# theori-io/nrsc5

Measured on AMD Instinct MI355X. Metric: IQ MS/s demod+decoded, higher is better.
Workload: dtype exact float32 half-band (== int16 Q15) / f32 OFDM + sync / int32 Viterbi metrics

## Files before the change

### nrsc5_amd/build.py

```python
from __future__ import annotations

import contextlib
import fcntl
import os
import subprocess
import sys

ROOT = os.path.dirname(os.path.dirname(os.path.abspath(__file__)))
CSRC = os.path.join(ROOT, "nrsc5_amd", "csrc")
HIP_SOURCES = ["engine.hip", "k_decimate.hip", "k_acquire.hip", "k_mixfft.hip", "k_sync.hip", "k_decode.hip", "k_replay.hip", "k_trim.hip", "k_am.hip", "k_l2.hip", "hdc_consumer.hip", "k_channelize.hip", "k_scan.hip"]
LIB = os.path.join(ROOT, "nrsc5_amd", "libnrsc5hip.so")
EMU_LIB = os.path.join(ROOT, "tests", "simt", "libnrsc5hip_emu.so")
HIPCC = os.environ.get("HIPCC", "/opt/rocm/bin/hipcc")


def _stale(target: str, deps) -> bool:
    if not os.path.exists(target):
        return True
    t = os.path.getmtime(target)
    return any(os.path.getmtime(d) > t for d in deps)


def _deps():
    d = [os.path.join(CSRC, f) for f in os.listdir(CSRC)]
    d.append(os.path.join(ROOT, "include", "nrsc5hip.h"))
    return d


@contextlib.contextmanager
def _build_lock(target: str):
    fd = os.open(os.path.dirname(target), os.O_RDONLY)
    try:
        fcntl.flock(fd, fcntl.LOCK_EX)
        yield
    finally:
        os.close(fd)


def _compile_to(target: str, cmd_for) -> None:
    tmp = "%s.tmp%d" % (target, os.getpid())
    try:
        subprocess.check_call(cmd_for(tmp))
        os.replace(tmp, target)
    finally:
        if os.path.exists(tmp):
            os.unlink(tmp)


def source_sha() -> str:
    import hashlib
    h = hashlib.sha256()
    for f in sorted(_deps()):
        if f.endswith((".hip", ".h")):
            h.update(os.path.basename(f).encode()); h.update(open(f, "rb").read())
    return h.hexdigest()[:16]


def build_hip(force: bool = False, verbose: bool = False) -> str:
    if force or _stale(LIB, _deps()):
        with _build_lock(LIB):
            if force or _stale(LIB, _deps()):
                srcs = [os.path.join(CSRC, f) for f in HIP_SOURCES if os.path.exists(os.path.join(CSRC, f))]

                def cmd(out):
                    c = [HIPCC, "--offload-arch=gfx950", "-O3", "-std=c++17", "-fPIC", "-shared", "-ffp-contract=off",
                         '-DNRSC5HIP_SOURCE_SHA="%s"' % source_sha(),
                         "-I" + os.path.join(ROOT, "include"), "-I" + CSRC, "-o", out] + srcs
                    if verbose:
                        print(" ".join(c))
                    return c
                _compile_to(LIB, cmd)
    return LIB


def build_hip_diag(flags, out_name: str) -> str:
    out = os.path.join(ROOT, "nrsc5_amd", out_name)
    srcs = [os.path.join(CSRC, f) for f in HIP_SOURCES if os.path.exists(os.path.join(CSRC, f))]
    cmd = [HIPCC, "--offload-arch=gfx950", "-O3", "-std=c++17", "-fPIC", "-shared", "-ffp-contract=off", '-DNRSC5HIP_SOURCE_SHA="%s"' % source_sha(),
           "-I" + os.path.join(ROOT, "include"), "-I" + CSRC, "-o", out] + list(flags) + srcs
    subprocess.check_call(cmd)
    return out


def _host_has_fma() -> bool:
    try:
        flags = next(l for l in open("/proc/cpuinfo") if l.startswith("flags")).split()
    except (OSError, StopIteration):
        return False
    return "fma" in flags


def build_emu(force: bool = False) -> str:
    simt = os.path.join(ROOT, "tests", "simt")
    deps = _deps() + [os.path.join(simt, "hipemu.h"), os.path.join(simt, "hipemu.cpp")]
    if force or _stale(EMU_LIB, deps):
        with _build_lock(EMU_LIB):
            if force or _stale(EMU_LIB, deps):
                srcs = [os.path.join(CSRC, f) for f in HIP_SOURCES if os.path.exists(os.path.join(CSRC, f))]
                fma = ["-mfma"] if _host_has_fma() else []

                def cmd(out):
                    c = ["g++", "-O2", "-g", "-std=c++17", "-fPIC", "-shared", "-ffp-contract=off", "-w"] + fma + ['-DNRSC5HIP_SOURCE_SHA="%s"' % source_sha(),
                         "-I" + simt, "-I" + os.path.join(ROOT, "include"), "-I" + CSRC, "-o", out,
                         os.path.join(simt, "hipemu.cpp")]
                    for s in srcs:
                        c += ["-x", "c++", s]
                    return c
                _compile_to(EMU_LIB, cmd)
    return EMU_LIB


if __name__ == "__main__":
    if "--emu" in sys.argv:
        print(build_emu(force=True))
    elif "--accurate-trig" in sys.argv:
        print(build_hip_diag(["-DNRSC5HIP_ACCURATE_TRIG"], "libnrsc5hip_acctrig.so"))
    elif "--cmul-unfused" in sys.argv:
        print(build_hip_diag(["-DNRSC5HIP_CMUL_UNFUSED"], "libnrsc5hip_unfused.so"))
    elif "--mixfft-noload" in sys.argv:
        print(build_hip_diag(["-DNRSC5HIP_MIXFFT_NOLOAD"], "libnrsc5hip_noload.so"))
    elif "--mixfft-phases" in sys.argv:
        print(build_hip_diag(["-DNRSC5HIP_MIXFFT_PHASES"], "libnrsc5hip_mixphases.so"))
    else:
        print(build_hip(force=True, verbose=True))
```

### nrsc5_amd/csrc/k_decode.hip

```cpp
#include <hip/hip_runtime.h>
#include "kernels.h"
#include "viterbi_wave.h"
#include "viterbi_v3.h"
#include "l2_header.h"

namespace nrsc5 {

__device__ inline int stream_of(const int *ids, int idx) { return ids ? ids[idx] : idx; }

__global__ __launch_bounds__(256) void k_p1_deint(DevTables tb, DevBuffers db, const int *ids, int parity, int lane_id)
{
    const int s = stream_of(ids, blockIdx.y);
    StreamState &st = db.state[s];
    if (!st.p1_pending[parity]) return;
    __shared__ uint32_t tile[16 * 180];
    __shared__ uint16_t lut[384];
    const int r = blockIdx.x, tid = threadIdx.x;
    const int8_t *pm = db.pm + ((size_t)s * NPM + st.p1_pmslot[parity]) * PM_FRAME;
    uint32_t *out = (uint32_t *)(db.coded + ((size_t)lane_id * db.nstreams_alloc + s) * P1_LEN);
    for (int w = tid; w < 16 * 180; w += 256) {
        const int b = w / 180, x = w % 180;
        tile[w] = ((const uint32_t *)(pm + ((size_t)b * 32 + r) * 720))[x];
    }
    for (int q = tid; q < 384; q += 256) lut[q] = tb.deint_lut[q];
    __syncthreads();
    const uint8_t *bytes = (const uint8_t *)tile;
    const int k0 = (3 * r) & 31;
    const int nk = (P1_CODED / 320 - k0 + 31) / 32;
    for (int idx = tid; idx < nk * 128; idx += 256) {
        const int m = idx >> 7, i = idx & 127;
        const int k = k0 + 32 * m;
        const int col = (11 * k + k / 288) % 36;
        uint32_t v = 0;
#pragma unroll
        for (int t = 0; t < 3; t++) {
            const unsigned off = lut[3 * i + t];
            if (off != 0xffffu) v |= (uint32_t)bytes[off + col] << (8 * t);
        }
        out[128 * k + i] = v;
    }
}

__device__ inline int bit_errors_k7_at(const int *soft, const uint32_t *bits, int len, int i)
{
    unsigned r = 0;
#pragma unroll
    for (int k = 0; k < 7; k++) {
        int q = i - k; if (q < 0) q += len;
        r |= ((bits[q >> 5] >> (q & 31)) & 1u) << (6 - k);
    }
    const int w = soft[i];
    const int c0 = (int8_t)w, c1 = (int8_t)(w >> 8), c2 = (int8_t)(w >> 16);
    const int p0 = __popc(r & 0133u) & 1, p1 = __popc(r & 0171u) & 1, p2 = __popc(r & 0165u) & 1;
    return ((c0 > 0) != p0) + ((c1 > 0) != p1) + (((i & 1) == 0) && ((c2 > 0) != p2));
}

__device__ inline int bit_errors_k7_partial(const int *soft, const uint32_t *bits, int len)
{
    int errors = 0;
    for (int i = threadIdx.x; i < len; i += blockDim.x) {
        unsigned r = 0;
#pragma unroll
        for (int k = 0; k < 7; k++) {
            int q = i - k; if (q < 0) q += len;
            r |= ((bits[q >> 5] >> (q & 31)) & 1u) << (6 - k);
        }
        const int w = soft[i];
        const int c0 = (int8_t)w, c1 = (int8_t)(w >> 8), c2 = (int8_t)(w >> 16);
        const int p0 = __popc(r & 0133u) & 1, p1 = __popc(r & 0171u) & 1, p2 = __popc(r & 0165u) & 1;
        if ((c0 > 0) != p0) errors++;
        if ((c1 > 0) != p1) errors++;
        if ((i & 1) == 0 && ((c2 > 0) != p2)) errors++;
    }
    return errors;
}

constexpr int FWD_WAVES = 4;
__global__ __launch_bounds__(64 * FWD_WAVES) void k_p1_forward(DevTables tb, DevBuffers db, const int *ids, int parity, int lane_id, int prio, int nstreams, int G, int warm)
{
    wave_set_priority(prio);
    const int widx = wave_uniform((int)(blockIdx.x * FWD_WAVES + (threadIdx.x >> 6)));
    if (widx >= nstreams * G) return;
    const int sidx = widx / G, g = widx % G;
    const int s = wave_uniform(stream_of(ids, sidx));
    StreamState &st = db.state[s];
    if (!st.p1_pending[parity]) return;
    const size_t slot = (size_t)lane_id * db.nstreams_alloc + s;
    const int *soft = db.coded + slot * P1_LEN;
    uint32_t *dec = db.dec + slot * (size_t)(2 * (P1_LEN + 64));
    viterbi3_forward_segment(soft, P1_LEN, dec, db.fwd_meta + slot * (size_t)(VIT3_GMAX * VIT3_META), g, G, warm);
}

__global__ __launch_bounds__(64 * FWD_WAVES) void k_p1_fix(DevTables tb, DevBuffers db, const int *ids, int parity, int lane_id, int prio, int nstreams, int G)
{
    wave_set_priority(prio);
    const int sidx = wave_uniform((int)(blockIdx.x * FWD_WAVES + (threadIdx.x >> 6)));
    if (sidx >= nstreams) return;
    const int s = wave_uniform(stream_of(ids, sidx));
    StreamState &st = db.state[s];
    if (!st.p1_pending[parity]) return;
    const size_t slot = (size_t)lane_id * db.nstreams_alloc + s;
    const int endlane = viterbi3_forward_fix(db.coded + slot * P1_LEN, P1_LEN, db.dec + slot * (size_t)(2 * (P1_LEN + 64)),
                                             db.fwd_meta + slot * (size_t)(VIT3_GMAX * VIT3_META), G, db.fwd_stats);
    if ((threadIdx.x & 63) == 0) st.p1_endlane[parity] = endlane;
}

constexpr int TB_THREADS = 1024;
constexpr int TBM_WAVES = 4;

__global__ __launch_bounds__(64 * TBM_WAVES) void k_p1_tbmap(DevTables tb, DevBuffers db, const int *ids, int parity, int lane_id, int prio, int parts)
{
    wave_set_priority(prio);
    const int s = stream_of(ids, blockIdx.y);
    StreamState &st = db.state[s];
    if (!st.p1_pending[parity]) return;
    const size_t slot = (size_t)lane_id * db.nstreams_alloc + s;
    viterbi3_traceback_maps(db.dec + slot * (size_t)(2 * (P1_LEN + 64)), P1_LEN, db.tbmap + slot * ((size_t)(P1_LEN / 64 + 1) * 64),
                            (int)(blockIdx.x * TBM_WAVES + (threadIdx.x >> 6)), parts * TBM_WAVES);
}

__global__ __launch_bounds__(64) void k_p1_tbwalk(DevTables tb, DevBuffers db, const int *ids, int parity, int lane_id, int prio, int nparts, int ntasks)
{
    wave_set_priority(prio);
    __shared__ uint32_t lds[TB2_LDS_WORDS];
    for (int t = (int)blockIdx.x; t < ntasks; t += (int)gridDim.x) {
        const int s = wave_uniform(stream_of(ids, t / nparts));
        StreamState &st = db.state[s];
        if (!st.p1_pending[parity]) continue;
        const size_t slot = (size_t)lane_id * db.nstreams_alloc + s;
        uint32_t *out = db.p1_ring + ((size_t)s * db.p1_slots + st.p1_slot[parity]) * P1_WORDS;
        viterbi3_traceback_walk(db.dec + slot * (size_t)(2 * (P1_LEN + 64)), P1_LEN, st.p1_endlane[parity], out,
                                db.tbmap + slot * ((size_t)(P1_LEN / 64 + 1) * 64), t % nparts, lds, db.coded + slot * P1_LEN);
        WAVE_LDS_FENCE();
    }
}

__global__ __launch_bounds__(TB_THREADS) void k_p1_traceback(DevTables tb, DevBuffers db, const int *ids, int parity, int lane_id, int l2_mode, int prio, int maps_done)
{
    wave_set_priority(prio);
    const int s = stream_of(ids, blockIdx.x);
    StreamState &st = db.state[s];
    if (!st.p1_pending[parity]) return;
    HIP_DYNAMIC_SHARED(uint8_t, smem)
    __shared__ int err_total;
    const int tid = threadIdx.x;
    const int *soft = db.coded + ((size_t)lane_id * db.nstreams_alloc + s) * P1_LEN;
    uint32_t *dec = db.dec + ((size_t)lane_id * db.nstreams_alloc + s) * (size_t)(2 * (P1_LEN + 64));
    uint32_t *out = db.p1_ring + ((size_t)s * db.p1_slots + st.p1_slot[parity]) * P1_WORDS;
    if (tid == 0) err_total = 0;
    uint8_t *gmap = db.tbmap + ((size_t)lane_id * db.nstreams_alloc + s) * ((size_t)(P1_LEN / 64 + 1) * 64);
    if (maps_done == 2) viterbi3_traceback_check(dec, P1_LEN, out, gmap, db.tb_stats, soft);
    else viterbi3_traceback_block(dec, P1_LEN, st.p1_endlane[parity], out, gmap, smem, maps_done != 0);
    __threadfence_block();
    __syncthreads();
    int errors;
    if (maps_done == 2) {
        constexpr int NCH = P1_LEN / 64 + 1;
        errors = 0;
        for (int c = tid; c < NCH; c += blockDim.x) errors += gmap[2 * NCH + c];
        if (tid < 6) errors += bit_errors_k7_at(soft, out, P1_LEN, tid);
        errors = wave_sum_i32(errors);
    } else {
        errors = wave_sum_i32(bit_errors_k7_partial(soft, out, P1_LEN));
    }
    if ((tid & 63) == 0) atomicAdd(&err_total, errors);
    __syncthreads();
    uint32_t *mirror = db.p1_mirror ? db.p1_mirror + ((size_t)s * db.p1_slots + st.p1_slot[parity]) * P1_WORDS : nullptr;
    for (int w = tid; w < P1_WORDS; w += blockDim.x) {
        const uint32_t v = out[w] ^ tb.scr_p1[w];
        out[w] = v;
        if (mirror) mirror[w] = v;
    }
    __threadfence_block();
    __syncthreads();
    __shared__ L2Smem l2;
    const bool ok = l2_mode ? l2_first_header_ok_fm_block(out, l2) : true;
    if (tid == 0) {
        BlockRecord &rec = db.records[(size_t)s * db.rec_cap + st.p1_record[parity]];
        rec.ber = (float)err_total / P1_CODED;
        if (l2_mode == 1) { if (!ok && st.sync_state == SYNC_FINE) { st.sync_state = SYNC_NONE; rec.state_after = SYNC_NONE; rec.flags |= REC_LOST_SYNC; } }
        else if (l2_mode) { __threadfence(); st.p1_verdict[parity] = ok ? 1 : 2; }
        if (db.l2_ring) st.p1_l2slot[parity] = st.p1_slot[parity] + 1;
        st.p1_pending[parity] = 0;
    }
}

static size_t traceback_smem(int len) { return vit3_traceback_smem(len); }

void launch_p1_deint(const DevTables &tb, const DevBuffers &db, int nstreams, const int *stream_ids, int parity, int lane_id, hipStream_t st)
{
    hipLaunchKernelGGL(k_p1_deint, dim3(32, nstreams), dim3(256), 0, st, tb, db, stream_ids, parity, lane_id);
}
void launch_p1_forward(const DevTables &tb, const DevBuffers &db, int nstreams, const int *stream_ids, int parity, int lane_id, hipStream_t st, int segments, int warm)
{
    constexpr int prio_fwd = 0;
    const int G = vit3_segments(P1_LEN, segments);
    hipLaunchKernelGGL(k_p1_forward, dim3((nstreams * G + FWD_WAVES - 1) / FWD_WAVES), dim3(64 * FWD_WAVES), 0, st, tb, db, stream_ids, parity, lane_id, prio_fwd, nstreams, G, warm);
    hipLaunchKernelGGL(k_p1_fix, dim3((nstreams + FWD_WAVES - 1) / FWD_WAVES), dim3(64 * FWD_WAVES), 0, st, tb, db, stream_ids, parity, lane_id, prio_fwd, nstreams, G);
}
void launch_p1_traceback(const DevTables &tb, const DevBuffers &db, int nstreams, const int *stream_ids, int parity, int lane_id, hipStream_t st, int l2_mode, int parts, int walk)
{
    constexpr int prio_tb = 1;
    if (walk) {
        const int nparts = vit3_tb2_waves(P1_LEN), ntasks = nparts * nstreams;
        const int grid = walk > 1 ? (walk < ntasks ? walk : ntasks) : ntasks;
        hipLaunchKernelGGL(k_p1_tbwalk, dim3(grid), dim3(64), 0, st, tb, db, stream_ids, parity, lane_id, prio_tb, nparts, ntasks);
        hipLaunchKernelGGL(k_p1_traceback, dim3(nstreams), dim3(TB_THREADS), traceback_smem(P1_LEN), st, tb, db, stream_ids, parity, lane_id, l2_mode, prio_tb, 2);
    } else {
        const int split = parts >= 16 ? 16 : 0;
        if (split) hipLaunchKernelGGL(k_p1_tbmap, dim3(split, nstreams), dim3(64 * TBM_WAVES), 0, st, tb, db, stream_ids, parity, lane_id, prio_tb, split);
        hipLaunchKernelGGL(k_p1_traceback, dim3(nstreams), dim3(TB_THREADS), traceback_smem(P1_LEN), st, tb, db, stream_ids, parity, lane_id, l2_mode, prio_tb, split ? 1 : 0);
    }
    if (db.l2_ring) launch_l2_index_window(db, nstreams, stream_ids, parity, st);
}

__global__ void k_stage_first_header(const uint32_t *words, int nwords, int am, int *ok)
{
    __shared__ L2Smem l2;
    const uint32_t *w = words + (size_t)blockIdx.x * nwords;
    const bool v = am ? l2_first_header_ok_am_block(w, l2) : l2_first_header_ok_fm_block(w, l2);
    if (threadIdx.x == 0) ok[blockIdx.x] = v ? 1 : 0;
}
void launch_stage_first_header(const uint32_t *words, int nwords, int nframes, int am, int threads, int *ok, hipStream_t st)
{
    hipLaunchKernelGGL(k_stage_first_header, dim3(nframes), dim3(threads), 0, st, words, nwords, am, ok);
}

__global__ __launch_bounds__(64) void k_viterbi_frames(const int8_t *coded, int len, unsigned long long *dec, uint32_t *out, int phases)
{
    const int f = blockIdx.x;
    viterbi_k7_decode(coded + (size_t)f * 3 * len, len, dec + (size_t)f * (len + 64), out + (size_t)f * ((len + 31) / 32), phases);
}
__global__ void k_pack_soft3(const int8_t *coded, int *soft, size_t nsteps)
{
    const size_t i = (size_t)blockIdx.x * blockDim.x + threadIdx.x;
    if (i >= nsteps) return;
    soft[i] = (int)(uint8_t)coded[3 * i] | ((int)(uint8_t)coded[3 * i + 1] << 8) | ((int)(uint8_t)coded[3 * i + 2] << 16);
}
__global__ __launch_bounds__(64) void k_viterbi_frames_fwd(const int *soft, int len, uint32_t *dec, int *meta, int G, int warm)
{
    const int f = blockIdx.x / G, g = blockIdx.x % G;
    viterbi3_forward_segment(soft + (size_t)f * len, len, dec + (size_t)f * 2 * (len + 64), meta + (size_t)f * VIT3_GMAX * VIT3_META, g, G, warm);
}
__global__ __launch_bounds__(64) void k_viterbi_frames_fix(const int *soft, int len, uint32_t *dec, int *meta, int G, int *endlane, int *stats)
{
    const int f = blockIdx.x;
    const int e = viterbi3_forward_fix(soft + (size_t)f * len, len, dec + (size_t)f * 2 * (len + 64), meta + (size_t)f * VIT3_GMAX * VIT3_META, G, stats);
    if ((threadIdx.x & 63) == 0) endlane[f] = e;
}
__global__ __launch_bounds__(64 * TBM_WAVES) void k_viterbi_frames_tbmap(uint32_t *dec, int len, uint8_t *gmap, int parts)
{
    const int f = blockIdx.y;
    viterbi3_traceback_maps(dec + (size_t)f * 2 * (len + 64), len, gmap + (size_t)f * (len / 64 + 1) * 64, (int)(blockIdx.x * TBM_WAVES + (threadIdx.x >> 6)), parts * TBM_WAVES);
}
__global__ __launch_bounds__(TB_THREADS) void k_viterbi_frames_tb(uint32_t *dec, int len, const int *endlane, uint32_t *out, uint8_t *gmap, int maps_done)
{
    HIP_DYNAMIC_SHARED(uint8_t, smem)
    const int f = blockIdx.x;
    viterbi3_traceback_block(dec + (size_t)f * 2 * (len + 64), len, endlane[f], out + (size_t)f * ((len + 31) / 32), gmap + (size_t)f * (len / 64 + 1) * 64, smem, maps_done != 0);
}

__global__ __launch_bounds__(64) void k_viterbi_frames_tbwalk(const uint32_t *dec, int len, const int *endlane, uint32_t *out, uint8_t *gmap)
{
    __shared__ uint32_t lds[TB2_LDS_WORDS];
    const int f = blockIdx.y;
    viterbi3_traceback_walk(dec + (size_t)f * 2 * (len + 64), len, endlane[f], out + (size_t)f * ((len + 31) / 32), gmap + (size_t)f * (len / 64 + 1) * 64, (int)blockIdx.x, lds);
}
__global__ __launch_bounds__(TB_THREADS) void k_viterbi_frames_tbcheck(const uint32_t *dec, int len, uint32_t *out, uint8_t *gmap, int *stats)
{
    const int f = blockIdx.x;
    viterbi3_traceback_check(dec + (size_t)f * 2 * (len + 64), len, out + (size_t)f * ((len + 31) / 32), gmap + (size_t)f * (len / 64 + 1) * 64, stats);
}

void vit_scratch_free(VitScratch &sc)
{
    if (sc.endlane) (void)hipFree(sc.endlane);
    if (sc.gmap) (void)hipFree(sc.gmap);
    if (sc.soft) (void)hipFree(sc.soft);
    if (sc.meta) (void)hipFree(sc.meta);
    sc = VitScratch();
}

template <typename T, typename N> static bool vit_grow(T *&p, N &cap, N need, size_t elem)
{
    if (cap >= need) return true;
    if (p) { (void)hipFree(p); p = nullptr; cap = 0; }
    if (hipMalloc((void **)&p, elem * (size_t)need) != hipSuccess) { p = nullptr; return false; }
    cap = need;
    return true;
}

static_assert((P1_LEN / 64 + 1 + TB_SEG - 1) / TB_SEG <= 64, "P1 frame exceeds the traceback's segment table");
constexpr int VIT3_MAX_LEN = (64 * TB_SEG - 1) * 64;

int launch_viterbi_frames(VitScratch &sc, const int8_t *coded, int len, int nframes, unsigned long long *dec, uint32_t *out, hipStream_t st, int phases, int segments, int *stats, int warm)
{
    if ((len & 63) == 0 && !(phases & 4)) {
        if (len > VIT3_MAX_LEN) return -1;
        int *&endlane = sc.endlane; uint8_t *&gmap = sc.gmap; int *&soft = sc.soft; int *&meta = sc.meta;
        const int cap_before = sc.cap;
        if (!vit_grow(endlane, sc.cap, nframes, sizeof(int))) return -1;
        if (sc.cap != cap_before) (void)hipMemsetAsync(endlane, 0, sizeof(int) * nframes, st);
        if (!vit_grow(meta, sc.mcap, nframes, sizeof(int) * (size_t)VIT3_GMAX * VIT3_META)) return -1;
        if (!vit_grow(gmap, sc.gcap, (size_t)nframes * (len / 64 + 1) * 64, 1)) return -1;
        if (!vit_grow(soft, sc.scap, (size_t)nframes * len, sizeof(int))) return -1;
        const size_t nsteps = (size_t)nframes * len;
        if (phases & 1) {
            if (!(phases & 8))
                hipLaunchKernelGGL(k_pack_soft3, dim3((unsigned)((nsteps + 255) / 256)), dim3(256), 0, st, coded, soft, nsteps);
            const int G = vit3_segments(len, segments);
            hipLaunchKernelGGL(k_viterbi_frames_fwd, dim3(nframes * G), dim3(64), 0, st, (const int *)soft, len, (uint32_t *)dec, meta, G, warm);
            hipLaunchKernelGGL(k_viterbi_frames_fix, dim3(nframes), dim3(64), 0, st, (const int *)soft, len, (uint32_t *)dec, meta, G, endlane, stats);
        }
        if ((phases & 2) && !(phases & 16)) {
            hipLaunchKernelGGL(k_viterbi_frames_tbwalk, dim3(vit3_tb2_waves(len), nframes), dim3(64), 0, st, (const uint32_t *)dec, len, (const int *)endlane, out, gmap);
            hipLaunchKernelGGL(k_viterbi_frames_tbcheck, dim3(nframes), dim3(TB_THREADS), 0, st, (const uint32_t *)dec, len, out, gmap, stats ? stats + 2 : nullptr);
        } else if (phases & 2) {
            const int split = segments >= 16 ? 16 : 0;
            if (split) hipLaunchKernelGGL(k_viterbi_frames_tbmap, dim3(split, nframes), dim3(64 * TBM_WAVES), 0, st, (uint32_t *)dec, len, gmap, split);
            hipLaunchKernelGGL(k_viterbi_frames_tb, dim3(nframes), dim3(TB_THREADS), traceback_smem(len), st, (uint32_t *)dec, len, (const int *)endlane, out, gmap, split ? 1 : 0);
        }
        return 0;
    }
    hipLaunchKernelGGL(k_viterbi_frames, dim3(nframes), dim3(64), 0, st, coded, len, dec, out, phases & 3);
    return 0;
}

__global__ __launch_bounds__(64) void k_selftest(int *fail)
{
    const int lane = threadIdx.x & 63;
    int bad = 0;
    for (int rep = 0; rep < 4; rep++) {
        const int v = (lane * 2654435 + rep * 977) ^ (lane << 20);
        bad += lane_xor<1>(v) != __shfl_xor(v, 1);
        bad += lane_xor<2>(v) != __shfl_xor(v, 2);
        bad += lane_xor<4>(v) != __shfl_xor(v, 4);
        bad += lane_xor<8>(v) != __shfl_xor(v, 8);
        bad += lane_xor<16>(v) != __shfl_xor(v, 16);
        bad += lane_xor<32>(v) != __shfl_xor(v, 32);
        int w = wave_writelane_c<37>(v, 12345);
        bad += w != (lane == 37 ? 12345 : v);
        const int a = (int)0x00817f05, b = (int)0x00ff0103;
        bad += dot4_i8(a, b, 7) != 7 + 15 + 127 + 127;
    }
    atomicAdd(fail, bad);
}

void launch_selftest(int *fail, hipStream_t st) { hipLaunchKernelGGL(k_selftest, dim3(4), dim3(64), 0, st, fail); }

}
```

### nrsc5_amd/csrc/viterbi_v3.h

```cpp
#pragma once
#include "nrsc5_dev.h"
#include "wave_ops.h"
#include "viterbi_wave.h"
#ifndef HIPEMU
#include "viterbi_v3_asm.h"
#endif

namespace nrsc5 {

#ifdef HIPEMU
struct v16i { int v[16]; int &operator[](int i) { return v[i]; } const int &operator[](int i) const { return v[i]; } };
#else
typedef int v16i __attribute__((ext_vector_type(16)));
#endif

struct Vit3Const {
    int w[4];
    int wp[2], wq[2];
    int s0[6];
};

__device__ __forceinline__ unsigned vit3_logical_lane(unsigned phys) { return phys ^ (((phys >> 2) & 1u) * 3u); }

__device__ inline Vit3Const vit3_consts(unsigned phys)
{
    const unsigned L = vit3_logical_lane(phys & 63u);
    Vit3Const k;
#pragma unroll
    for (int r = 0; r < 6; r++) {
        const unsigned S = rotr6(L, r);
        const unsigned reg = S & 0x3eu;
        const int g0 = (__popc(reg & 0133u) & 1) ? 2 : -2, g1 = (__popc(reg & 0171u) & 1) ? 2 : -2, g2 = (__popc(reg & 0165u) & 1) ? 2 : -2;
        const int pos = (g0 & 0xff) | ((g1 & 0xff) << 8) | ((g2 & 0xff) << 16);
        const int neg = (-g0 & 0xff) | ((-g1 & 0xff) << 8) | ((-g2 & 0xff) << 16);
        k.s0[r] = (int)(S & 1u);
        if (r < 4) k.w[r] = pos;
        else {
            k.wp[r - 4] = (S & 1u) ? neg : pos;
            k.wq[r - 4] = (S & 1u) ? pos : neg;
        }
    }
    return k;
}

__device__ __forceinline__ int vit3_push(int hist, int ns)
{
#ifdef HIPEMU
    return (int)(((unsigned)hist >> 1) | ((unsigned)ns << 31));
#else
    return (int)__builtin_amdgcn_alignbit((unsigned)ns, (unsigned)hist, 1);
#endif
}

template <int R, bool PUSH>
__device__ __forceinline__ void vit3_step_c(int &u, int &hist, int &ns, int nsp, int aw, const Vit3Const &k)
{
    if (PUSH) hist = vit3_push(hist, nsp);
    if constexpr (R < 4) {
        const int D = dot4_i8(aw, k.w[R], 0);
        constexpr int M = R == 0 ? 1 : R == 1 ? 2 : R == 2 ? 7 : 8;
        const int X = u + D, Y = __shfl_xor(u, M) - D;
        ns = X > Y ? X : Y;
    } else {
        constexpr int M = R == 4 ? 16 : 32;
        const int P = dot4_i8(aw, k.wp[R - 4], u), Q = dot4_i8(aw, k.wq[R - 4], u);
        const int Pin = __shfl_xor(P, M), Qin = __shfl_xor(Q, M);
        const bool upper = (threadIdx.x & M) != 0;
        const int P2 = upper ? Qin : P, Q2 = upper ? Q : Pin;
        ns = P2 > Q2 ? P2 : Q2;
    }
    u = (ns & ~1) | k.s0[(R + 1) % 6];
}

#define V3_OPERANDS                                                                                                      \
    : [u] "+v"(u), [h] "+v"(hist), [ns] "+v"(ns), [x] "=&v"(x), [d0] "=&v"(d0), [d1] "=&v"(d1), [d2] "=&v"(d2), [d3] "=&v"(d3)   \
    : [a0] "s"(a0), [a1] "s"(a1), [a2] "s"(a2), [a3] "s"(a3), [a4] "s"(a4), [a5] "s"(a5), [a6] "s"(a6), [a7] "s"(a7),   \
      [w0] "v"(k.w[0]), [w1] "v"(k.w[1]), [w2] "v"(k.w[2]), [w3] "v"(k.w[3]),                                           \
      [p4] "v"(k.wp[0]), [q4] "v"(k.wq[0]), [p5] "v"(k.wp[1]), [q5] "v"(k.wq[1]),                                       \
      [z0] "v"(k.s0[0]), [z1] "v"(k.s0[1]), [z2] "v"(k.s0[2]), [z3] "v"(k.s0[3]), [z4] "v"(k.s0[4]), [z5] "v"(k.s0[5])

template <int PH, bool W0>
__device__ __forceinline__ void vit3_block8(int &u, int &hist, int &ns, int a0, int a1, int a2, int a3, int a4, int a5, int a6, int a7, const Vit3Const &k)
{
    static_assert(PH == 0 || PH == 2 || PH == 4, "8-step blocks start in an even phase");
#ifdef HIPEMU
    int na;
    vit3_step_c<(PH + 0) % 6, !W0>(u, hist, na, ns, a0, k);
    vit3_step_c<(PH + 1) % 6, true>(u, hist, ns, na, a1, k);
    vit3_step_c<(PH + 2) % 6, true>(u, hist, na, ns, a2, k);
    vit3_step_c<(PH + 3) % 6, true>(u, hist, ns, na, a3, k);
    vit3_step_c<(PH + 4) % 6, true>(u, hist, na, ns, a4, k);
    vit3_step_c<(PH + 5) % 6, true>(u, hist, ns, na, a5, k);
    vit3_step_c<(PH + 6) % 6, true>(u, hist, na, ns, a6, k);
    vit3_step_c<(PH + 7) % 6, true>(u, hist, ns, na, a7, k);
#else
    int x, d0, d1, d2, d3;
    if constexpr (PH == 0) { if constexpr (W0) asm(VIT3_ASM_PH0_OPEN V3_OPERANDS); else asm(VIT3_ASM_PH0_CONT V3_OPERANDS); }
    else if constexpr (PH == 2) { if constexpr (W0) asm(VIT3_ASM_PH2_OPEN V3_OPERANDS); else asm(VIT3_ASM_PH2_CONT V3_OPERANDS); }
    else { if constexpr (W0) asm(VIT3_ASM_PH4_OPEN V3_OPERANDS); else asm(VIT3_ASM_PH4_CONT V3_OPERANDS); }
#endif
}

template <int PH, bool W0>
__device__ __forceinline__ void vit3_run16(int &u, int &hist, int &nsp, const v16i &a, const Vit3Const &k)
{
    vit3_block8<PH, W0>(u, hist, nsp, a[0], a[1], a[2], a[3], a[4], a[5], a[6], a[7], k);
    vit3_block8<(PH + 8) % 6, false>(u, hist, nsp, a[8], a[9], a[10], a[11], a[12], a[13], a[14], a[15], k);
}

__device__ __forceinline__ v16i vit3_load16(const int *p)
{
#ifdef HIPEMU
    v16i v;
    for (int i = 0; i < 16; i++) v[i] = p[i];
    return v;
#else
    typedef const __attribute__((address_space(4))) v16i *cptr;
    return *(cptr)(uintptr_t)p;
#endif
}

constexpr int VIT3_WARM = 6;
#ifdef HIPEMU
__device__ inline void vit3_keep(int) {}
#else
__device__ __forceinline__ void vit3_keep(int v) { asm volatile("" :: "v"(v)); }
#endif
#ifdef HIPEMU
#define VIT3_SCHED_BARRIER() do { } while (0)
#define VIT3_WAIT_SCALAR() do { } while (0)
#else
#define VIT3_SCHED_BARRIER() __builtin_amdgcn_sched_barrier(0)
#define VIT3_WAIT_SCALAR() do { __builtin_amdgcn_sched_barrier(0); __builtin_amdgcn_s_waitcnt(0xc07f); __builtin_amdgcn_sched_barrier(0); } while (0)
#endif

template <int PH>
__device__ __forceinline__ void vit3_word(int &u, int &hist, int &nsp, const v16i &c0, const v16i &c1, v16i &n0, v16i &n1,
                                          const int *soft, int len, int &jn, const Vit3Const &k, uint32_t *&dec_word)
{
    VIT3_WAIT_SCALAR();
    n0 = vit3_load16(soft + jn); n1 = vit3_load16(soft + jn + 16);
    jn += 32; if (jn >= len) jn -= len;
    VIT3_SCHED_BARRIER();
    vit3_run16<PH, true>(u, hist, nsp, c0, k);
    vit3_run16<(PH + 16) % 6, false>(u, hist, nsp, c1, k);
    hist = vit3_push(hist, nsp);
    *dec_word = (uint32_t)hist;
    dec_word += 64;
}

constexpr int VIT3_WARM_TRIPS = 2;

__device__ __host__ inline int vit3_trips(int len) { return (len / 64 + 1) / 3; }
__device__ __host__ inline int vit3_segments(int len, int want)
{
    const int T = vit3_trips(len);
    int g = want < 1 ? 1 : want > VIT3_GMAX ? VIT3_GMAX : want;
    while (g > 1 && T / g < VIT3_WARM_TRIPS + 1) g--;
    return g;
}

__device__ __forceinline__ int viterbi3_forward_span(const int *soft, int len, uint32_t *dec, uint32_t *scratch, int trip0, int trip1, int warm,
                                                      bool last, bool have_u0, int u0, int *snap, int *uend)
{
    const unsigned phys = threadIdx.x & 63u, L = vit3_logical_lane(phys);
    const Vit3Const k = vit3_consts(phys);
    const int nchunks = len / 64 + 1;
    const int tstart = trip0 - warm;
    int u = (have_u0 && !warm) ? u0 : k.s0[0], hist = 0, nsp = 0;
    int jn = (len - VIT_EXTRA + 192 * tstart) % len;
    int jw = (jn + 64 * VIT3_WARM) % len, warmv = 0;
    v16i a0 = vit3_load16(soft + jn), a1 = vit3_load16(soft + jn + 16), b0, b1;
    jn += 32; if (jn >= len) jn -= len;
    uint32_t *w = dec + (size_t)384 * trip0 + L;
    for (int t = tstart; t < trip1; t++) {
        if (warm) {
            if (t < trip0) w = scratch + L;
            else if (t == trip0) { snap[L] = u; w = dec + (size_t)384 * trip0 + L; }
        }
        int jl = jw + (int)phys; if (jl >= len) jl -= len;
        const int w0 = soft[jl], w1 = soft[jl + 64 < len ? jl + 64 : jl + 64 - len], w2 = soft[jl + 128 < len ? jl + 128 : jl + 128 - len];
        jw += 192; if (jw >= len) jw -= len;
        vit3_word<0>(u, hist, nsp, a0, a1, b0, b1, soft, len, jn, k, w);
        vit3_word<2>(u, hist, nsp, b0, b1, a0, a1, soft, len, jn, k, w);
        vit3_word<4>(u, hist, nsp, a0, a1, b0, b1, soft, len, jn, k, w);
        vit3_word<0>(u, hist, nsp, b0, b1, a0, a1, soft, len, jn, k, w);
        vit3_word<2>(u, hist, nsp, a0, a1, b0, b1, soft, len, jn, k, w);
        vit3_word<4>(u, hist, nsp, b0, b1, a0, a1, soft, len, jn, k, w);
        warmv ^= w0 ^ w1 ^ w2;
    }
    if (last) {
        const int rest = nchunks % 3;
        if (rest >= 1) {
            vit3_word<0>(u, hist, nsp, a0, a1, b0, b1, soft, len, jn, k, w);
            vit3_word<2>(u, hist, nsp, b0, b1, a0, a1, soft, len, jn, k, w);
        }
        if (rest == 2) {
            vit3_word<4>(u, hist, nsp, a0, a1, b0, b1, soft, len, jn, k, w);
            vit3_word<0>(u, hist, nsp, b0, b1, a0, a1, soft, len, jn, k, w);
        }
    }
    vit3_keep(warmv);
    if (uend) uend[L] = u;
    return u;
}

__device__ __forceinline__ int vit3_end_lane(int u, int len)
{
    const unsigned L = vit3_logical_lane(threadIdx.x & 63u);
    const int nchunks = len / 64 + 1;
    const int rend = (64 * nchunks) % 6;
    const int pm = u >> 1;
    const int best = wave_max_i32(pm);
    const int smin = wave_min_i32(pm == best ? (int)rotr6(L, rend) : 64);
    return wave_uniform((int)rotl6((unsigned)smin, rend));
}

__device__ __forceinline__ void viterbi3_forward_segment(const int *soft, int len, uint32_t *dec, int *meta, int g, int G, int warm)
{
    const int T = vit3_trips(len);
    int *m = meta + (size_t)g * VIT3_META;
    if (g && !warm) m[vit3_logical_lane(threadIdx.x & 63u)] = (int)(rotr6(vit3_logical_lane(threadIdx.x & 63u), 0) & 1u);
    viterbi3_forward_span(soft, len, dec, (uint32_t *)(m + 128), g * T / G, (g + 1) * T / G, g ? warm : 0, g == G - 1, false, 0, m, m + 64);
}

__device__ __forceinline__ int viterbi3_forward_fix(const int *soft, int len, uint32_t *dec, int *meta, int G, int *stats)
{
    const unsigned L = vit3_logical_lane(threadIdx.x & 63u);
    const int T = vit3_trips(len);
    int repaired = 0;
    int ue = meta[64 + L];
    for (int g = 1; g < G; g++) {
        int *m = meta + (size_t)g * VIT3_META;
        const int sn = m[L];
        const int d = (ue - wave_uniform(ue)) - (sn - wave_uniform(sn));
        if (wave_max_i32(d < 0 ? -d : d) != 0) {
            ue = viterbi3_forward_span(soft, len, dec, nullptr, g * T / G, (g + 1) * T / G, 0, g == G - 1, true, ue, nullptr, m + 64);
            repaired++;
        } else {
            ue = m[64 + L];
        }
    }
    if (stats && (threadIdx.x & 63) == 0) { atomicAdd(&stats[0], G - 1); if (repaired) atomicAdd(&stats[1], repaired); }
    return vit3_end_lane(ue, len);
}

__device__ __forceinline__ int viterbi3_forward(const int *soft, int len, uint32_t *dec)
{
    const int u = viterbi3_forward_span(soft, len, dec, nullptr, 0, vit3_trips(len), 0, true, false, 0, nullptr, nullptr);
    return vit3_end_lane(u, len);
}

__device__ __forceinline__ unsigned vit3_fetch_lane(unsigned l4, unsigned v)
{
#ifdef HIPEMU
    return (unsigned)__shfl((int)v, (int)(l4 >> 2));
#else
    return (unsigned)__builtin_amdgcn_ds_bpermute((int)l4, (int)v);
#endif
}

template <int PHA, int PHB, int S> struct Vit3Map2 {
    static __device__ __forceinline__ void run(unsigned &la, unsigned h0a, unsigned h1a, unsigned &ahia, unsigned &aloa,
                                               unsigned &lb, unsigned h0b, unsigned h1b, unsigned &ahib, unsigned &alob)
    {
        constexpr int RA = (PHA + S) % 6, RB = (PHB + S) % 6;
        const unsigned va = vit3_fetch_lane(la, S >= 32 ? h1a : h0a), vb = vit3_fetch_lane(lb, S >= 32 ? h1b : h0b);
        const unsigned da = (va >> (S & 31)) & 1u, db = (vb >> (S & 31)) & 1u;
        if (S >= 32) { ahia = (ahia << 1) | da; ahib = (ahib << 1) | db; } else { aloa = (aloa << 1) | da; alob = (alob << 1) | db; }
        la = (la & ~(4u << RA)) | (da << (RA + 2));
        lb = (lb & ~(4u << RB)) | (db << (RB + 2));
        Vit3Map2<PHA, PHB, S - 1>::run(la, h0a, h1a, ahia, aloa, lb, h0b, h1b, ahib, alob);
    }
};
template <int PHA, int PHB> struct Vit3Map2<PHA, PHB, -1> {
    static __device__ __forceinline__ void run(unsigned &, unsigned, unsigned, unsigned &, unsigned &, unsigned &, unsigned, unsigned, unsigned &, unsigned &) {}
};

template <int PH>
__device__ __forceinline__ void vit3_outputs(unsigned lane, unsigned ahi, unsigned alo, unsigned &ohi, unsigned &olo)
{
    unsigned top = 0;
#pragma unroll
    for (int k = 0; k < 6; k++) top |= ((lane >> ((PH + 58 + k) % 6)) & 1u) << k;
    ohi = (ahi >> 6) | (top << 26);
    olo = (alo >> 6) | (ahi << 26);
}

__device__ __host__ inline size_t vit3_traceback_smem(int len)
{
    const int nchunks = len / 64 + 1, nseg = (nchunks + TB_SEG - 1) / TB_SEG;
    return (size_t)nseg * 64 + (size_t)nchunks;
}

__device__ __forceinline__ void viterbi3_traceback_maps(uint32_t *dec, int len, uint8_t *gmap, int gw, int nw)
{
    const int lane = threadIdx.x & 63;
    const int nchunks = len / 64 + 1;
    for (int ca = 2 * gw; ca < nchunks; ca += 2 * nw) {
        const int cb = ca + 1;
        const bool two = cb < nchunks;
        const unsigned h0a = dec[(size_t)(2 * ca) * 64 + lane], h1a = dec[(size_t)(2 * ca + 1) * 64 + lane];
        const unsigned h0b = two ? dec[(size_t)(2 * cb) * 64 + lane] : 0u, h1b = two ? dec[(size_t)(2 * cb + 1) * 64 + lane] : 0u;
        unsigned la = (unsigned)lane << 2, lb = la, ahia = 0, aloa = 0, ahib = 0, alob = 0, ohia, oloa, ohib, olob;
        switch (ca % 3) {
        case 0: Vit3Map2<0, 4, 63>::run(la, h0a, h1a, ahia, aloa, lb, h0b, h1b, ahib, alob);
                vit3_outputs<0>((unsigned)lane, ahia, aloa, ohia, oloa); vit3_outputs<4>((unsigned)lane, ahib, alob, ohib, olob); break;
        case 1: Vit3Map2<4, 2, 63>::run(la, h0a, h1a, ahia, aloa, lb, h0b, h1b, ahib, alob);
                vit3_outputs<4>((unsigned)lane, ahia, aloa, ohia, oloa); vit3_outputs<2>((unsigned)lane, ahib, alob, ohib, olob); break;
        default: Vit3Map2<2, 0, 63>::run(la, h0a, h1a, ahia, aloa, lb, h0b, h1b, ahib, alob);
                vit3_outputs<2>((unsigned)lane, ahia, aloa, ohia, oloa); vit3_outputs<0>((unsigned)lane, ahib, alob, ohib, olob); break;
        }
        gmap[64 * ca + lane] = (uint8_t)(la >> 2);
        dec[(size_t)(2 * ca) * 64 + lane] = oloa; dec[(size_t)(2 * ca + 1) * 64 + lane] = ohia;
        if (two) {
            gmap[64 * cb + lane] = (uint8_t)(lb >> 2);
            dec[(size_t)(2 * cb) * 64 + lane] = olob; dec[(size_t)(2 * cb + 1) * 64 + lane] = ohib;
        }
    }
}

__device__ inline void viterbi3_traceback_block(uint32_t *dec, int len, int endlane, uint32_t *out, uint8_t *gmap, uint8_t *smem, bool maps_done = false)
{
    const int tid = threadIdx.x, lane = tid & 63, wave = tid >> 6, nwaves = blockDim.x >> 6;
    const int nchunks = len / 64 + 1, nseg = (nchunks + TB_SEG - 1) / TB_SEG;
    uint8_t *segmap = smem, *chosen = smem + (size_t)nseg * 64;
    __shared__ uint8_t segend[64];
    if (!maps_done) viterbi3_traceback_maps(dec, len, gmap, wave, nwaves);
    __threadfence_block();
    __syncthreads();
    for (int sg = wave; sg < nseg; sg += nwaves) {
        const int c0 = sg * TB_SEG, c1 = min(nchunks, c0 + TB_SEG);
        unsigned e = (unsigned)lane;
        for (int c = c1 - 1; c >= c0; c--) e = gmap[64 * c + e];
        segmap[64 * sg + lane] = (uint8_t)e;
    }
    __syncthreads();
    if (tid == 0) {
        unsigned e = (unsigned)endlane;
        for (int sg = nseg - 1; sg >= 0; sg--) { segend[sg] = (uint8_t)e; e = segmap[64 * sg + e]; }
    }
    __syncthreads();
    for (int sg = tid; sg < nseg; sg += blockDim.x) {
        const int c0 = sg * TB_SEG, c1 = min(nchunks, c0 + TB_SEG);
        unsigned e = segend[sg];
        for (int c = c1 - 1; c >= c0; c--) { chosen[c] = (uint8_t)e; e = gmap[64 * c + e]; }
    }
    __syncthreads();
    for (int c = tid; c < nchunks; c += blockDim.x) {
        if (c < nchunks - 1) out[2 * c] = dec[(size_t)(2 * c + 1) * 64 + chosen[c]];
        if (c >= 1) out[2 * c - 1] = dec[(size_t)(2 * c) * 64 + chosen[c]];
    }
}

constexpr int TB2_CHUNKS = 64;
constexpr int TB2_LDS_WORDS = (TB2_CHUNKS + 1) * 128;
__device__ __host__ inline int vit3_tb2_waves(int len) { return ((len / 64 + 1) + TB2_CHUNKS - 1) / TB2_CHUNKS; }
__device__ __host__ inline size_t vit3_tb2_meta_bytes(int len) { return (size_t)3 * (len / 64 + 1); }

__device__ __forceinline__ void vit3_walk_rotated(const uint32_t *rows, unsigned &q, unsigned &ahi, unsigned &alo)
{
    ahi = 0; alo = 0;
#pragma unroll
    for (int S = 63; S >= 0; S--) {
        const int u = S % 6;
        const unsigned v = rows[(S >= 32 ? 64 : 0) + q];
        const unsigned d = (v >> (S & 31)) & 1u;
        if (S >= 32) ahi |= d << (S & 31); else alo |= d << (S & 31);
        q = (q & ~(1u << u)) | (d << u);
    }
}

__device__ __forceinline__ void vit3_outputs_rotated(unsigned qend, unsigned ahi, unsigned alo, unsigned &ohi, unsigned &olo)
{
    unsigned top = 0;
#pragma unroll
    for (int k = 0; k < 6; k++) top |= ((qend >> ((58 + k) % 6)) & 1u) << k;
    ohi = (ahi >> 6) | (top << 26);
    olo = (alo >> 6) | (ahi << 26);
}

__device__ __forceinline__ unsigned vit3_chunk_errors(const int *soft, int len, int c, unsigned prev6, unsigned olo, unsigned ohi)
{
    const unsigned long long wlo = (unsigned long long)prev6 | ((unsigned long long)olo << 6) | ((unsigned long long)ohi << 38);
    const unsigned whi = ohi >> 26;
    unsigned errors = 0;
    for (int S = 0; S < 64; S++) {
        const int i = 64 * c + S - VIT_EXTRA;
        if (i < 6 || i >= len) continue;
        const unsigned r = (unsigned)((S <= 57 ? (wlo >> S) : ((wlo >> S) | ((unsigned long long)whi << (64 - S)))) & 0x7full);
        const int w = soft[i];
        const int c0 = (int8_t)w, c1 = (int8_t)(w >> 8), c2 = (int8_t)(w >> 16);
        const int p0 = __popc(r & 0133u) & 1, p1 = __popc(r & 0171u) & 1, p2 = __popc(r & 0165u) & 1;
        errors += ((c0 > 0) != p0) + ((c1 > 0) != p1) + (((i & 1) == 0) && ((c2 > 0) != p2));
    }
    return errors;
}
__device__ __forceinline__ unsigned vit3_prev6(int c, unsigned exit_lane)
{
    const int php = (4 * ((c + 2) % 3)) % 6;
    unsigned v = 0;
#pragma unroll
    for (int k = 0; k < 6; k++) v |= ((exit_lane >> ((php + 58 + k) % 6)) & 1u) << k;
    return v;
}

__device__ __forceinline__ void viterbi3_traceback_walk(const uint32_t *dec, int len, int endlane, uint32_t *out, uint8_t *meta, int w, uint32_t *lds, const int *soft = nullptr)
{
    const int lane = threadIdx.x & 63;
    const int nchunks = len / 64 + 1;
    const int c0 = w * TB2_CHUNKS, nrows = min(TB2_CHUNKS + 1, nchunks - c0);
    for (int i = lane; i < nrows * 128; i += 64) {
        const int k = i >> 7, h = (i >> 6) & 1, L = i & 63;
        const int ph = (4 * ((c0 + k) % 3)) % 6;
        lds[128 * k + 64 * h + (int)rotr6((unsigned)L, ph)] = dec[(size_t)(2 * (c0 + k) + h) * 64 + L];
    }
    WAVE_LDS_SYNC();
    const int c = c0 + lane;
    if (c >= nchunks) return;
    const int ph = (4 * (c % 3)) % 6;
    unsigned q, ahi, alo;
    if (c == nchunks - 1) {
        q = rotr6((unsigned)endlane, ph);
    } else {
        unsigned qa = 0, t0, t1;
        vit3_walk_rotated(lds + 128 * (lane + 1), qa, t0, t1);
        q = rotl6(qa, 4);
    }
    const unsigned qend = q;
    vit3_walk_rotated(lds + 128 * lane, q, ahi, alo);
    unsigned ohi, olo;
    vit3_outputs_rotated(qend, ahi, alo, ohi, olo);
    if (c < nchunks - 1) out[2 * c] = ohi;
    if (c >= 1) out[2 * c - 1] = olo;
    meta[c] = (uint8_t)rotl6(qend, ph);
    const unsigned lexit = rotl6(q, ph);
    meta[nchunks + c] = (uint8_t)lexit;
    if (soft) meta[2 * nchunks + c] = (uint8_t)vit3_chunk_errors(soft, len, c, vit3_prev6(c, lexit), olo, ohi);
}

__device__ inline unsigned vit3_rewalk(const uint32_t *dec, int c, unsigned e, unsigned &ohi, unsigned &olo)
{
    const int ph = (4 * (c % 3)) % 6;
    unsigned l = e, ahi = 0, alo = 0;
    for (int S = 63; S >= 0; S--) {
        const int R = (ph + S) % 6;
        const unsigned v = dec[(size_t)(2 * c + (S >> 5)) * 64 + l];
        const unsigned d = (v >> (S & 31)) & 1u;
        if (S >= 32) ahi |= d << (S & 31); else alo |= d << (S & 31);
        l = (l & ~(1u << R)) | (d << R);
    }
    unsigned top = 0;
    for (int k = 0; k < 6; k++) top |= ((e >> ((ph + 58 + k) % 6)) & 1u) << k;
    ohi = (ahi >> 6) | (top << 26);
    olo = (alo >> 6) | (ahi << 26);
    return l;
}

__device__ inline void viterbi3_traceback_check(const uint32_t *dec, int len, uint32_t *out, uint8_t *meta, int *stats, const int *soft = nullptr)
{
    const int nchunks = len / 64 + 1;
    __shared__ int tb2_bad;
    int rewalked = 0;
    for (int round = 0; round <= nchunks; round++) {
        if (threadIdx.x == 0) tb2_bad = 0;
        __syncthreads();
        int mine[4]; unsigned want[4]; int nm = 0;
        for (int c = threadIdx.x; c < nchunks - 1; c += blockDim.x) {
            const unsigned w = meta[nchunks + c + 1];
            if (meta[c] != w && nm < 4) { mine[nm] = c; want[nm] = w; nm++; }
        }
        if (nm) tb2_bad = 1;
        __syncthreads();
        if (!tb2_bad) break;
        for (int k = 0; k < nm; k++) {
            const int c = mine[k];
            unsigned ohi, olo;
            const unsigned l = vit3_rewalk(dec, c, want[k], ohi, olo);
            out[2 * c] = ohi;
            if (c >= 1) out[2 * c - 1] = olo;
            meta[c] = (uint8_t)want[k]; meta[nchunks + c] = (uint8_t)l;
            if (soft) meta[2 * nchunks + c] = (uint8_t)vit3_chunk_errors(soft, len, c, vit3_prev6(c, l), olo, ohi);
            rewalked++;
        }
        __threadfence_block();
        __syncthreads();
    }
    if (stats) { if (threadIdx.x == 0) atomicAdd(&stats[0], nchunks - 1); if (rewalked) atomicAdd(&stats[1], rewalked); }
}

}
```

Baseline: 248,000.

## Vectorize traceback-walk tile loads and compute chunk errors via ballot re-encoding

The traceback walk now loads the decision tile as uint4 slices, and prefetches soft symbols alongside it. It computes per-chunk bit errors by re-encoding the decoded bits and comparing against received hard decisions collected with wave ballots, replacing the per-chunk scalar error routine. The check kernel launches without dynamic LDS, and its per-thread mismatch capacity is sized from the thread count. An optional run-in length knob and a phase-timing diagnostic build are added. These changes aim to cut global-load and error-count latency in traceback, at the cost of more registers and more complex indexing.

```diff
diff --git a/nrsc5_amd/build.py b/nrsc5_amd/build.py
--- a/nrsc5_amd/build.py
+++ b/nrsc5_amd/build.py
@@ -121,5 +121,7 @@
         print(build_hip_diag(["-DNRSC5HIP_MIXFFT_NOLOAD"], "libnrsc5hip_noload.so"))
     elif "--mixfft-phases" in sys.argv:
         print(build_hip_diag(["-DNRSC5HIP_MIXFFT_PHASES"], "libnrsc5hip_mixphases.so"))
+    elif "--tbwalk-phases" in sys.argv:
+        print(build_hip_diag(["-DNRSC5HIP_TBWALK_PHASES"], "libnrsc5hip_tbphases.so"))
     else:
         print(build_hip(force=True, verbose=True))
diff --git a/nrsc5_amd/csrc/k_decode.hip b/nrsc5_amd/csrc/k_decode.hip
--- a/nrsc5_amd/csrc/k_decode.hip
+++ b/nrsc5_amd/csrc/k_decode.hip
@@ -106,6 +106,12 @@
 }
 
 constexpr int TB_THREADS = 1024;
+#ifndef NRSC5HIP_TBC_THREADS
+#define NRSC5HIP_TBC_THREADS 1024
+#endif
+constexpr int TBC_THREADS = NRSC5HIP_TBC_THREADS;
+constexpr int TBC_NM = (P1_LEN / 64 + 1 + TBC_THREADS - 1) / TBC_THREADS;
+static_assert(TBC_THREADS % 64 == 0 && TBC_THREADS >= 64 && TBC_THREADS <= TB_THREADS, "check workgroup: whole waves, within k_p1_traceback's launch bound");
 constexpr int TBM_WAVES = 4;
 
 __global__ __launch_bounds__(64 * TBM_WAVES) void k_p1_tbmap(DevTables tb, DevBuffers db, const int *ids, int parity, int lane_id, int prio, int parts)
@@ -119,6 +125,11 @@
                             (int)(blockIdx.x * TBM_WAVES + (threadIdx.x >> 6)), parts * TBM_WAVES);
 }
 
+#ifdef NRSC5HIP_TBWALK_PHASES
+#define TBWALK_PHASE_CYCLES(db) ((db).sync_phase_cycles ? (db).sync_phase_cycles + 8 : nullptr)
+#else
+#define TBWALK_PHASE_CYCLES(db) nullptr
+#endif
 __global__ __launch_bounds__(64) void k_p1_tbwalk(DevTables tb, DevBuffers db, const int *ids, int parity, int lane_id, int prio, int nparts, int ntasks)
 {
     wave_set_priority(prio);
@@ -130,7 +141,7 @@
         const size_t slot = (size_t)lane_id * db.nstreams_alloc + s;
         uint32_t *out = db.p1_ring + ((size_t)s * db.p1_slots + st.p1_slot[parity]) * P1_WORDS;
         viterbi3_traceback_walk(db.dec + slot * (size_t)(2 * (P1_LEN + 64)), P1_LEN, st.p1_endlane[parity], out,
-                                db.tbmap + slot * ((size_t)(P1_LEN / 64 + 1) * 64), t % nparts, lds, db.coded + slot * P1_LEN);
+                                db.tbmap + slot * ((size_t)(P1_LEN / 64 + 1) * 64), t % nparts, lds, db.coded + slot * P1_LEN, TBWALK_PHASE_CYCLES(db));
         WAVE_LDS_FENCE();
     }
 }
@@ -149,7 +160,7 @@
     uint32_t *out = db.p1_ring + ((size_t)s * db.p1_slots + st.p1_slot[parity]) * P1_WORDS;
     if (tid == 0) err_total = 0;
     uint8_t *gmap = db.tbmap + ((size_t)lane_id * db.nstreams_alloc + s) * ((size_t)(P1_LEN / 64 + 1) * 64);
-    if (maps_done == 2) viterbi3_traceback_check(dec, P1_LEN, out, gmap, db.tb_stats, soft);
+    if (maps_done == 2) viterbi3_traceback_check<TBC_NM>(dec, P1_LEN, out, gmap, db.tb_stats, soft);
     else viterbi3_traceback_block(dec, P1_LEN, st.p1_endlane[parity], out, gmap, smem, maps_done != 0);
     __threadfence_block();
     __syncthreads();
@@ -205,7 +216,7 @@
         const int nparts = vit3_tb2_waves(P1_LEN), ntasks = nparts * nstreams;
         const int grid = walk > 1 ? (walk < ntasks ? walk : ntasks) : ntasks;
         hipLaunchKernelGGL(k_p1_tbwalk, dim3(grid), dim3(64), 0, st, tb, db, stream_ids, parity, lane_id, prio_tb, nparts, ntasks);
-        hipLaunchKernelGGL(k_p1_traceback, dim3(nstreams), dim3(TB_THREADS), traceback_smem(P1_LEN), st, tb, db, stream_ids, parity, lane_id, l2_mode, prio_tb, 2);
+        hipLaunchKernelGGL(k_p1_traceback, dim3(nstreams), dim3(TBC_THREADS), 0, st, tb, db, stream_ids, parity, lane_id, l2_mode, prio_tb, 2);
     } else {
         const int split = parts >= 16 ? 16 : 0;
         if (split) hipLaunchKernelGGL(k_p1_tbmap, dim3(split, nstreams), dim3(64 * TBM_WAVES), 0, st, tb, db, stream_ids, parity, lane_id, prio_tb, split);
diff --git a/nrsc5_amd/csrc/viterbi_v3.h b/nrsc5_amd/csrc/viterbi_v3.h
--- a/nrsc5_amd/csrc/viterbi_v3.h
+++ b/nrsc5_amd/csrc/viterbi_v3.h
@@ -358,11 +358,12 @@
 __device__ __host__ inline int vit3_tb2_waves(int len) { return ((len / 64 + 1) + TB2_CHUNKS - 1) / TB2_CHUNKS; }
 __device__ __host__ inline size_t vit3_tb2_meta_bytes(int len) { return (size_t)3 * (len / 64 + 1); }
 
-__device__ __forceinline__ void vit3_walk_rotated(const uint32_t *rows, unsigned &q, unsigned &ahi, unsigned &alo)
+template <int S0>
+__device__ __forceinline__ void vit3_walk_rotated_from(const uint32_t *rows, unsigned &q, unsigned &ahi, unsigned &alo)
 {
     ahi = 0; alo = 0;
 #pragma unroll
-    for (int S = 63; S >= 0; S--) {
+    for (int S = S0; S >= 0; S--) {
         const int u = S % 6;
         const unsigned v = rows[(S >= 32 ? 64 : 0) + q];
         const unsigned d = (v >> (S & 31)) & 1u;
@@ -370,6 +371,7 @@
         q = (q & ~(1u << u)) | (d << u);
     }
 }
+__device__ __forceinline__ void vit3_walk_rotated(const uint32_t *rows, unsigned &q, unsigned &ahi, unsigned &alo) { vit3_walk_rotated_from<63>(rows, q, ahi, alo); }
 
 __device__ __forceinline__ void vit3_outputs_rotated(unsigned qend, unsigned ahi, unsigned alo, unsigned &ohi, unsigned &olo)
 {
@@ -405,38 +407,116 @@
     return v;
 }
 
-__device__ __forceinline__ void viterbi3_traceback_walk(const uint32_t *dec, int len, int endlane, uint32_t *out, uint8_t *meta, int w, uint32_t *lds, const int *soft = nullptr)
+__device__ __forceinline__ void vit3_chunk_encode(unsigned prev6, unsigned olo, unsigned ohi, unsigned long long enc[3])
+{
+    const unsigned long long wlo = (unsigned long long)prev6 | ((unsigned long long)olo << 6) | ((unsigned long long)ohi << 38);
+    const unsigned long long whi = ohi >> 26;
+    unsigned long long sh[7];
+    sh[0] = wlo;
+#pragma unroll
+    for (int j = 1; j < 7; j++) sh[j] = (wlo >> j) | (whi << (64 - j));
+    const unsigned long long common = sh[0] ^ sh[4] ^ sh[6];
+    enc[0] = common ^ sh[1] ^ sh[3];
+    enc[1] = common ^ sh[3] ^ sh[5];
+    enc[2] = common ^ sh[2] ^ sh[5];
+}
+#ifndef NRSC5HIP_TB2_RUNIN
+#define NRSC5HIP_TB2_RUNIN 64
+#endif
+constexpr int TB2_RUNIN = NRSC5HIP_TB2_RUNIN;
+static_assert(TB2_RUNIN == 64 || TB2_RUNIN == 32, "run-in: a whole chunk or its lower history word");
+constexpr int TB2_SLICES = 4, TB2_SLICE_V4 = 9, TB2_SLICE_CHUNKS = TB2_CHUNKS / TB2_SLICES;
+static_assert(TB2_SLICES * TB2_SLICE_V4 * 64 * 4 >= TB2_LDS_WORDS && TB2_SLICES * TB2_SLICE_CHUNKS == TB2_CHUNKS, "the slices cover the tile");
+
+#ifdef NRSC5HIP_TBWALK_PHASES
+#define TB2_MARK_BEGIN long long tb2_t0 = (long long)clock64()
+#define TB2_MARK(i) do { __builtin_amdgcn_s_waitcnt(0); if (phase_cycles && (threadIdx.x & 63) == 0) { const long long now = (long long)clock64(); \
+    atomicAdd((unsigned long long *)&phase_cycles[i], (unsigned long long)(now - tb2_t0)); tb2_t0 = now; } } while (0)
+#else
+#define TB2_MARK_BEGIN do { } while (0)
+#define TB2_MARK(i) do { } while (0)
+#endif
+
+__device__ __forceinline__ void viterbi3_traceback_walk(const uint32_t *dec, int len, int endlane, uint32_t *out, uint8_t *meta, int w, uint32_t *lds, const int *soft = nullptr, long long *phase_cycles = nullptr)
 {
     const int lane = threadIdx.x & 63;
     const int nchunks = len / 64 + 1;
     const int c0 = w * TB2_CHUNKS, nrows = min(TB2_CHUNKS + 1, nchunks - c0);
-    for (int i = lane; i < nrows * 128; i += 64) {
-        const int k = i >> 7, h = (i >> 6) & 1, L = i & 63;
-        const int ph = (4 * ((c0 + k) % 3)) % 6;
-        lds[128 * k + 64 * h + (int)rotr6((unsigned)L, ph)] = dec[(size_t)(2 * (c0 + k) + h) * 64 + L];
+    TB2_MARK_BEGIN;
+    const uint4 *src = reinterpret_cast<const uint4 *>(dec + (size_t)128 * c0);
+    const int nv = nrows * 32;
+    int m3 = (c0 + (lane >> 5)) % 3;
+    int rx[6] = {0, 0, 0, 0, 0, 0};
+#pragma unroll 1
+    for (int sl = 0; sl < TB2_SLICES; sl++) {
+        uint4 piece[TB2_SLICE_V4];
+        int sw[TB2_SLICE_CHUNKS];
+#pragma unroll
+        for (int jj = 0; jj < TB2_SLICE_V4; jj++) piece[jj] = src[min(lane + 64 * (TB2_SLICE_V4 * sl + jj), nv - 1)];
+        if (soft) {
+#pragma unroll
+            for (int kk = 0; kk < TB2_SLICE_CHUNKS; kk++)
+                sw[kk] = soft[min(max(64 * (c0 + TB2_SLICE_CHUNKS * sl + kk) + lane - VIT_EXTRA, 0), len - 1)];
+        }
+#pragma unroll
+        for (int jj = 0; jj < TB2_SLICE_V4; jj++) {
+            const int i4 = lane + 64 * (TB2_SLICE_V4 * sl + jj);
+            const int ph = m3 == 0 ? 0 : m3 == 1 ? 4 : 2;
+            m3 = m3 == 0 ? 2 : m3 - 1;
+            if (i4 < nv) {
+                uint32_t *row = lds + 64 * (i4 >> 4);
+                const unsigned L = 4u * (unsigned)(i4 & 15);
+                row[(((L + 0) >> ph) | ((L + 0) << (6 - ph))) & 63u] = piece[jj].x;
+                row[(((L + 1) >> ph) | ((L + 1) << (6 - ph))) & 63u] = piece[jj].y;
+                row[(((L + 2) >> ph) | ((L + 2) << (6 - ph))) & 63u] = piece[jj].z;
+                row[(((L + 3) >> ph) | ((L + 3) << (6 - ph))) & 63u] = piece[jj].w;
+            }
+        }
+        if (soft) {
+#pragma unroll
+            for (int kk = 0; kk < TB2_SLICE_CHUNKS; kk++) {
+                const int k = TB2_SLICE_CHUNKS * sl + kk, v = sw[kk];
+                const unsigned long long b0 = __ballot((int8_t)v > 0), b1 = __ballot((int8_t)(v >> 8) > 0), b2 = __ballot((int8_t)(v >> 16) > 0);
+                rx[0] = wave_writelane(rx[0], (int)(unsigned)b0, k); rx[1] = wave_writelane(rx[1], (int)(unsigned)(b0 >> 32), k);
+                rx[2] = wave_writelane(rx[2], (int)(unsigned)b1, k); rx[3] = wave_writelane(rx[3], (int)(unsigned)(b1 >> 32), k);
+                rx[4] = wave_writelane(rx[4], (int)(unsigned)b2, k); rx[5] = wave_writelane(rx[5], (int)(unsigned)(b2 >> 32), k);
+            }
+        }
     }
     WAVE_LDS_SYNC();
+    TB2_MARK(0);
     const int c = c0 + lane;
-    if (c >= nchunks) return;
+    const bool own = c < nchunks;
     const int ph = (4 * (c % 3)) % 6;
-    unsigned q, ahi, alo;
-    if (c == nchunks - 1) {
-        q = rotr6((unsigned)endlane, ph);
-    } else {
-        unsigned qa = 0, t0, t1;
-        vit3_walk_rotated(lds + 128 * (lane + 1), qa, t0, t1);
-        q = rotl6(qa, 4);
-    }
-    const unsigned qend = q;
-    vit3_walk_rotated(lds + 128 * lane, q, ahi, alo);
-    unsigned ohi, olo;
-    vit3_outputs_rotated(qend, ahi, alo, ohi, olo);
-    if (c < nchunks - 1) out[2 * c] = ohi;
-    if (c >= 1) out[2 * c - 1] = olo;
-    meta[c] = (uint8_t)rotl6(qend, ph);
-    const unsigned lexit = rotl6(q, ph);
-    meta[nchunks + c] = (uint8_t)lexit;
-    if (soft) meta[2 * nchunks + c] = (uint8_t)vit3_chunk_errors(soft, len, c, vit3_prev6(c, lexit), olo, ohi);
+    unsigned ohi = 0, olo = 0, lexit = 0;
+    if (own) {
+        unsigned q, ahi, alo;
+        if (c == nchunks - 1) {
+            q = rotr6((unsigned)endlane, ph);
+        } else {
+            unsigned qa = 0, t0, t1;
+            vit3_walk_rotated_from<TB2_RUNIN - 1>(lds + 128 * (lane + 1), qa, t0, t1);
+            q = rotl6(qa, 4);
+        }
+        const unsigned qend = q;
+        vit3_walk_rotated(lds + 128 * lane, q, ahi, alo);
+        vit3_outputs_rotated(qend, ahi, alo, ohi, olo);
+        if (c < nchunks - 1) out[2 * c] = ohi;
+        if (c >= 1) out[2 * c - 1] = olo;
+        meta[c] = (uint8_t)rotl6(qend, ph);
+        lexit = rotl6(q, ph);
+        meta[nchunks + c] = (uint8_t)lexit;
+    }
+    TB2_MARK(1);
+    if (soft && own) {
+        const unsigned long long valid = (c == 0 ? ~0ull << (VIT_EXTRA + 6) : ~0ull) & (c == nchunks - 1 ? (1ull << VIT_EXTRA) - 1 : ~0ull);
+        unsigned long long enc[3];
+        vit3_chunk_encode(vit3_prev6(c, lexit), olo, ohi, enc);
+        const unsigned long long r0 = (unsigned)rx[0] | ((unsigned long long)(unsigned)rx[1] << 32), r1 = (unsigned)rx[2] | ((unsigned long long)(unsigned)rx[3] << 32),
+                                 r2 = (unsigned)rx[4] | ((unsigned long long)(unsigned)rx[5] << 32);
+        meta[2 * nchunks + c] = (uint8_t)(__popcll((r0 ^ enc[0]) & valid) + __popcll((r1 ^ enc[1]) & valid) + __popcll((r2 ^ enc[2]) & valid & 0x5555555555555555ull));
+    }
+    TB2_MARK(2);
 }
 
 __device__ inline unsigned vit3_rewalk(const uint32_t *dec, int c, unsigned e, unsigned &ohi, unsigned &olo)
@@ -457,6 +537,7 @@
     return l;
 }
 
+template <int NM = 4>
 __device__ inline void viterbi3_traceback_check(const uint32_t *dec, int len, uint32_t *out, uint8_t *meta, int *stats, const int *soft = nullptr)
 {
     const int nchunks = len / 64 + 1;
@@ -465,10 +546,10 @@
     for (int round = 0; round <= nchunks; round++) {
         if (threadIdx.x == 0) tb2_bad = 0;
         __syncthreads();
-        int mine[4]; unsigned want[4]; int nm = 0;
+        int mine[NM]; unsigned want[NM]; int nm = 0;
         for (int c = threadIdx.x; c < nchunks - 1; c += blockDim.x) {
             const unsigned w = meta[nchunks + c + 1];
-            if (meta[c] != w && nm < 4) { mine[nm] = c; want[nm] = w; nm++; }
+            if (meta[c] != w && nm < NM) { mine[nm] = c; want[nm] = w; nm++; }
         }
         if (nm) tb2_bad = 1;
         __syncthreads();
```

Result: faster. 273,100, median of 6 (+10.1%).
